# Nahuel-M/StereoVisionArray

Measured on AMD Instinct MI355X. Metric: Mdisparities/sec (W·H·D/s) at 1080p D=128, higher is better.
Workload: dtype u16

## Files before the change

### stereovisionarray_amd/csrc/sgm_common.h

```cpp
#pragma once

#include <utility>

#include "sva_device.h"
#include "sva_internal.h"
#include "sva_tuning.h"

namespace sva {
namespace sgm {

template <class F, int... S>
__device__ __forceinline__ void for_seq_impl(std::integer_sequence<int, S...>, F&& f) {
    (f(std::integral_constant<int, S>{}), ...);
}
template <int N, class F>
__device__ __forceinline__ void for_seq(F&& f) {
    for_seq_impl(std::make_integer_sequence<int, N>{}, static_cast<F&&>(f));
}

constexpr unsigned INF2 = 0x7fff7fffu;

struct PathGeom {
    int W, H, D;
    int P1, P2;
    int blk_h;
    int blk_w;
    size_t vol;
    int ckpt;
    int ns;
    size_t ckvol;
    int nsy;
    size_t ckvvol;
    int npair;
    size_t cstr, lstr, ckstr, ckvstr;
    int pair;
    int dreal;
};


typedef __amdgpu_buffer_rsrc_t rsrc_t;


constexpr int kStoreNT = 2;

__device__ __forceinline__ rsrc_t make_rsrc(const void* base, size_t bytes) {
    return __builtin_amdgcn_make_buffer_rsrc(const_cast<void*>(base), (short)0,
                                             (int)(unsigned)bytes, 0x00020000);
}

template <int NW>
struct Words {
    unsigned w[NW];
};

template <int NW, int AUX = tune::kCLoadAux>
__device__ __forceinline__ Words<NW> bload(rsrc_t r, unsigned off) {
    Words<NW> o;
    if constexpr (NW == 1) {
        o.w[0] = __builtin_amdgcn_raw_buffer_load_b32(r, off, 0, AUX);
    } else if constexpr (NW == 2) {
        auto v = __builtin_amdgcn_raw_buffer_load_b64(r, off, 0, AUX);
        o.w[0] = v[0]; o.w[1] = v[1];
    } else if constexpr (NW == 3) {
        auto v = __builtin_amdgcn_raw_buffer_load_b96(r, off, 0, AUX);
        o.w[0] = v[0]; o.w[1] = v[1]; o.w[2] = v[2];
    } else {
        auto v = __builtin_amdgcn_raw_buffer_load_b128(r, off, 0, AUX);
        o.w[0] = v[0]; o.w[1] = v[1]; o.w[2] = v[2]; o.w[3] = v[3];
    }
    return o;
}

template <int NW, int AUX = kStoreNT>
__device__ __forceinline__ void bstore(rsrc_t r, unsigned off, const unsigned (&w)[NW]) {
    if constexpr (NW == 1) {
        __builtin_amdgcn_raw_buffer_store_b32(w[0], r, off, 0, AUX);
    } else if constexpr (NW == 2) {
        typedef unsigned v2u __attribute__((ext_vector_type(2)));
        __builtin_amdgcn_raw_buffer_store_b64((v2u){w[0], w[1]}, r, off, 0, AUX);
    } else if constexpr (NW == 3) {
        typedef unsigned v3u __attribute__((ext_vector_type(3)));
        __builtin_amdgcn_raw_buffer_store_b96((v3u){w[0], w[1], w[2]}, r, off, 0, AUX);
    } else {
        typedef unsigned v4u __attribute__((ext_vector_type(4)));
        __builtin_amdgcn_raw_buffer_store_b128((v4u){w[0], w[1], w[2], w[3]}, r, off, 0, AUX);
    }
}

__device__ __forceinline__ unsigned add3(unsigned a, unsigned b, unsigned c) {
    unsigned r;
    asm("v_add3_u32 %0, %1, %2, %3" : "=v"(r) : "v"(a), "v"(b), "v"(c));
    return r;
}

template <bool DIAG>
struct Cursor {
    int x;
    unsigned off;
    __device__ __forceinline__ bool advance(int rx, unsigned stride, int W, unsigned WD) {
        off += stride;
        if constexpr (DIAG) {
            x += rx;
            const bool hi = x >= W, lo = x < 0;
            x = hi ? x - W : (lo ? x + W : x);
            off = hi ? off - WD : (lo ? off + WD : off);
            return hi || lo;
        }
        return false;
    }
};

__device__ __forceinline__ unsigned min3_u16x2(unsigned a, unsigned b, unsigned c) {
    unsigned r;
    asm("v_pk_minimum3_f16 %0, %1, %2, %3" : "=v"(r) : "v"(a), "v"(b), "v"(c));
    return r;
}

template <int NP>
__device__ __forceinline__ unsigned lane_min_u16(const unsigned (&A)[NP]) {
    unsigned mm[NP];
#pragma unroll
    for (int j = 0; j < NP; j++) mm[j] = A[j];
    int n = NP;
#pragma unroll
    for (int it = 0; it < 4; it++) {
        if (n > 1) {
            int o = 0, i = 0;
#pragma unroll
            for (int q = 0; q < 8; q++) {
                if (i + 2 < n) { mm[o++] = min3_u16x2(mm[i], mm[i + 1], mm[i + 2]); i += 3; }
                else if (i + 1 < n) { mm[o++] = as_u32(vmin2(as_v2(mm[i]), as_v2(mm[i + 1]))); i += 2; }
                else if (i < n) { mm[o++] = mm[i]; i += 1; }
            }
            n = o;
        }
    }
    const u16x2 mf = as_v2(mm[0]);
    return mf.x < mf.y ? mf.x : mf.y;
}

template <int DPL> __host__ __device__ constexpr int pair_d(int j, int h) {
    return tune::kSplitPairs ? j + h * (DPL / 2) : 2 * j + h;
}
template <int DPL> __host__ __device__ constexpr int pair_of(int e) {
    return tune::kSplitPairs ? e % (DPL / 2) : e >> 1;
}
template <int DPL> __host__ __device__ constexpr int half_of(int e) {
    return tune::kSplitPairs ? e / (DPL / 2) : e & 1;
}

template <int DPL>
__device__ __forceinline__ void words_to_pairs(const unsigned (&w)[DPL / 4], unsigned (&A)[DPL / 2]) {
    constexpr int NW = DPL / 4, NP = DPL / 2;
    if constexpr (tune::kSplitPairs != 0) {
#pragma unroll
        for (int j = 0; j < NP; j++) {
            constexpr unsigned Z = 0x0cu;
            const int el = j, eh = j + NP;
            const unsigned sel = (unsigned)(el & 3) | (Z << 8) | ((4u + (unsigned)(eh & 3)) << 16) | (Z << 24);
            A[j] = __builtin_amdgcn_perm(w[eh >> 2], w[el >> 2], sel);
        }
    } else {
#pragma unroll
        for (int q = 0; q < NW; q++) unpack4(w[q], A[2 * q], A[2 * q + 1]);
    }
}

template <int DPL>
__device__ __forceinline__ void pairs_to_words(const unsigned (&A)[DPL / 2], unsigned (&ow)[DPL / 4]) {
    constexpr int NW = DPL / 4, NP = DPL / 2;
    if constexpr (tune::kSplitPairs != 0) {
        unsigned T[NP / 2];
#pragma unroll
        for (int i = 0; i < NP / 2; i++) T[i] = __builtin_amdgcn_perm(A[2 * i + 1], A[2 * i], 0x06020400u);
        if constexpr (NP == 2) {
            ow[0] = T[0];
        } else {
#pragma unroll
            for (int q = 0; q < NW; q++) {
                const int e0 = 4 * q, e2 = 4 * q + 2;
                const int a = (e0 % NP) / 2, ha = e0 / NP, b = (e2 % NP) / 2, hb = e2 / NP;
                const unsigned sel = (unsigned)(2 * ha) | ((unsigned)(2 * ha + 1) << 8) |
                                     ((unsigned)(4 + 2 * hb) << 16) | ((unsigned)(5 + 2 * hb) << 24);
                ow[q] = __builtin_amdgcn_perm(T[b], T[a], sel);
            }
        }
    } else {
#pragma unroll
        for (int w = 0; w < NW; w++) ow[w] = pack4(A[2 * w], A[2 * w + 1]);
    }
}

struct Edges {
    unsigned X = INF2, Y = INF2;
};

template <int DPL, bool PIN = false>
__device__ __forceinline__ void sgm_step_c(const unsigned (&c)[DPL / 2], unsigned (&A)[DPL / 2],
                                           unsigned& m, unsigned (&ow)[DPL / 4], unsigned P1,
                                           unsigned P2, Edges& e) {
    constexpr int NP = DPL / 2;
    e.X = row_shr1(A[NP - 1], e.X);
    e.Y = row_shl1(A[0], e.Y);
    const unsigned X = e.X, Y = e.Y;
    unsigned lo[NP], hi[NP];
    if constexpr (tune::kSplitPairs != 0) {
#pragma unroll
        for (int j = 0; j < NP; j++) {
            lo[j] = j == 0 ? __builtin_amdgcn_alignbit(A[NP - 1], X, 16) : A[j - 1];
            hi[j] = j == NP - 1 ? __builtin_amdgcn_alignbit(Y, A[0], 16) : A[j + 1];
        }
    } else {
        unsigned M[NP];
        M[0] = __builtin_amdgcn_alignbit(A[0], X, 16);
#pragma unroll
        for (int j = 1; j < NP; j++) M[j] = __builtin_amdgcn_alignbit(A[j], A[j - 1], 16);
        const unsigned Qlast = __builtin_amdgcn_alignbit(Y, A[NP - 1], 16);
#pragma unroll
        for (int j = 0; j < NP; j++) {
            lo[j] = M[j];
            hi[j] = j < NP - 1 ? M[j + 1] : Qlast;
        }
    }
    unsigned K, mP2;
    asm("v_mul_i32_i24_e32 %0, 0xfffeffff, %1" : "=v"(K) : "v"(m));
    if constexpr (tune::kStepMadP2 != 0) {
        asm("v_mad_u32_u24 %0, %1, %2, %3" : "=&v"(mP2) : "v"(m), "s"(0x10001u), "v"(P2 * 0x10001u));
    } else {
        mP2 = P2 * 0x10001u - K;
    }
    u16x2 t[NP];
#pragma unroll
    for (int j = 0; j < NP; j++) t[j] = vmin2(as_v2(lo[j]), as_v2(hi[j]));
    unsigned tp[NP];
    if constexpr (tune::kStepAddU32 != 0) {
        const unsigned P1x2 = P1 * 0x10001u;
#pragma unroll
        for (int j = 0; j < NP; j++) tp[j] = as_u32(t[j]) + P1x2;
    } else {
#pragma unroll
        for (int j = 0; j < NP; j++) tp[j] = as_u32(t[j] + splat2(P1));
    }
#pragma unroll
    for (int j = 0; j < NP; j++) A[j] = add3(min3_u16x2(tp[j], A[j], mP2), c[j], K);
    pairs_to_words<DPL>(A, ow);
    m = row_min_u32<PIN>(lane_min_u16<NP>(A));
}

template <int DPL>
__device__ __forceinline__ void sgm_step_c(const unsigned (&c)[DPL / 2], unsigned (&A)[DPL / 2],
                                           unsigned& m, unsigned (&ow)[DPL / 4], unsigned P1,
                                           unsigned P2) {
    Edges e;
    sgm_step_c<DPL>(c, A, m, ow, P1, P2, e);
}

template <int DPL, bool PIN = false>
__device__ __forceinline__ void sgm_step(const unsigned (&cw)[DPL / 4], unsigned (&A)[DPL / 2],
                                         unsigned& m, unsigned (&ow)[DPL / 4], unsigned P1,
                                         unsigned P2, Edges& e) {
    unsigned c[DPL / 2];
    words_to_pairs<DPL>(cw, c);
    sgm_step_c<DPL, PIN>(c, A, m, ow, P1, P2, e);
}

__device__ __forceinline__ void dir_of(int r, int& rx, int& ry) {
    constexpr int T[8][2] = {{1, 0}, {-1, 0}, {0, 1}, {0, -1}, {1, 1}, {-1, -1}, {-1, 1}, {1, -1}};
    rx = T[r][0];
    ry = T[r][1];
}

template <int DPL> constexpr int pf_h() {
    return DPL == 4 ? tune::kPfH4 : DPL == 8 ? tune::kPfH8 : DPL == 12 ? tune::kPfH12 : tune::kPfH16;
}
template <int DPL> constexpr int pf_v() {
    return DPL == 4 ? tune::kPfV4 : DPL == 8 ? tune::kPfV8 : DPL == 12 ? tune::kPfV12 : tune::kPfV16;
}


template <int DPL, bool DIAG, int PF, int CKPT = 0, int SL = 0>
__device__ __forceinline__ void path_line(rsrc_t rC, rsrc_t rL, const PathGeom& g, int rx, int ry,
                                          int line, int k, rsrc_t rCK) {
    constexpr int NW = DPL / 4, NP = DPL / 2;
    const int W = g.W, H = g.H, D = g.D;
    const unsigned P1 = (unsigned)g.P1, P2 = (unsigned)g.P2;
    const int steps = ry == 0 ? W : H;
    const unsigned WD = (unsigned)W * (unsigned)D;
    const unsigned stride = (unsigned)((ry * W + rx) * D);
    int x0, y0;
    if (ry == 0) { y0 = line; x0 = rx > 0 ? 0 : W - 1; }
    else { y0 = ry > 0 ? 0 : H - 1; x0 = line; }
    Cursor<false> cc;
    cc.x = x0;
    cc.off = ((unsigned)y0 * (unsigned)W + (unsigned)x0) * (unsigned)D + (unsigned)(k * DPL);
    Cursor<false> pc = cc;
    constexpr bool STATIC_HITS = DPL <= tune::kStaticCkptHitsMaxDpl && (CKPT == 1 || CKPT == 2) &&
                                 SL > 0 && PF % (1 << SL) == 0;
    int lead = 0;
    if constexpr (STATIC_HITS) {
        constexpr int SEG = 1 << SL;
        lead = CKPT == 1 ? (rx > 0 ? 0 : (SEG - W % SEG) % SEG) : (ry > 0 ? 0 : (SEG - H % SEG) % SEG);
        pc.off -= (unsigned)lead * stride;
    }
    const int nsteps = steps + lead;
    int twc = 0, twp = 0, Tc = 0, Tp = 0;
    if constexpr (DIAG) {
        const int j = (int)((threadIdx.x >> 4) & 3);
        const int l0 = __builtin_amdgcn_readfirstlane(line - j);
        twc = twp = rx > 0 ? W - line : line + 1;
        Tc = Tp = rx > 0 ? W - l0 - 3 : l0 + 1;
    }
    const bool narrow = W < 4;

    unsigned A[NP];
#pragma unroll
    for (int j = 0; j < NP; j++) A[j] = 0u;
    unsigned m = 0u;
    Edges edges;

    Words<NW> ring[PF];
#pragma unroll
    for (int p = 0; p < PF; p++) {
        ring[p] = bload<NW>(rC, pc.off);
        if constexpr (STATIC_HITS) {
#pragma unroll
            for (int w = 0; w < NW; w++) ring[p].w[w] = p < lead ? 0u : ring[p].w[w];
        }
        pc.off += stride;
        if constexpr (DIAG) {
            if (p < PF - 1) {
                const bool w = p + 1 == twp;
                const unsigned fixed = rx > 0 ? pc.off - WD : pc.off + WD;
                pc.off = w ? fixed : pc.off;
                twp = w ? twp + W : twp;
            }
        }
    }
    if constexpr (DIAG) {
        while (Tp + 3 < PF) Tp += W;
    }

    auto step = [&](int p, bool refill, int ts) {
        unsigned cw[NW];
#pragma unroll
        for (int w = 0; w < NW; w++) cw[w] = ring[p].w[w];
        unsigned ow[NW];
        sgm_step<DPL>(cw, A, m, ow, P1, P2, edges);
        if constexpr (CKPT == 1 && STATIC_HITS) {
            constexpr int SEG = 1 << SL;
            if ((p & (SEG - 1)) == SEG - 1) {
                const int x = rx > 0 ? ts : W - 1 - (ts - lead);
                if (rx > 0 ? x + 1 < W : x > 0)
                    bstore<NW, tune::kCkptStoreAux>(rCK, ((unsigned)(y0 * g.ns + (x >> SL)) * (unsigned)D +
                                             (unsigned)(k * DPL)), ow);
            }
        } else if constexpr (CKPT == 2 && STATIC_HITS) {
            constexpr int SEG = 1 << SL;
            if ((p & (SEG - 1)) == SEG - 1) {
                const int y = ry > 0 ? ts : H - 1 - (ts - lead);
                if (ry > 0 ? y + 1 < H : y > 0)
                    bstore<NW, tune::kCkptStoreAux>(rCK, ((unsigned)((y >> SL) * W + x0) * (unsigned)D +
                                             (unsigned)(k * DPL)), ow);
            }
        } else if constexpr (CKPT == 1) {
            const int x = rx > 0 ? ts : W - 1 - ts;
            constexpr int SEG = 1 << SL;
            const bool hit = rx > 0 ? (((x + 1) & (SEG - 1)) == 0 && x + 1 < W)
                                    : ((x & (SEG - 1)) == 0 && x > 0);
            if (__builtin_expect(hit, 0))
                bstore<NW, tune::kCkptStoreAux>(rCK, ((unsigned)(y0 * g.ns + (x >> SL)) * (unsigned)D +
                                         (unsigned)(k * DPL)), ow);
        } else if constexpr (CKPT == 3) {
            const int y = ry > 0 ? ts : H - 1 - ts;
            constexpr int SEG = 1 << SL;
            const bool hit = ry > 0 ? (((y + 1) & (SEG - 1)) == 0 && y + 1 < H)
                                    : ((y & (SEG - 1)) == 0 && y > 0);
            if (__builtin_expect(hit, 0))
                bstore<NW, tune::kCkptStoreAux>(rCK, cc.off - (unsigned)(y - (y >> SL)) * WD, ow);
        } else if constexpr (CKPT == 2) {
            const int y = ry > 0 ? ts : H - 1 - ts;
            constexpr int SEG = 1 << SL;
            const bool hit = ry > 0 ? (((y + 1) & (SEG - 1)) == 0 && y + 1 < H)
                                    : ((y & (SEG - 1)) == 0 && y > 0);
            if (__builtin_expect(hit, 0))
                bstore<NW, tune::kCkptStoreAux>(rCK, ((unsigned)((y >> SL) * W + x0) * (unsigned)D +
                                         (unsigned)(k * DPL)), ow);
        } else {
            bstore<NW>(rL, cc.off, ow);
        }
        cc.off += stride;
        if constexpr (DIAG) {
            const int ec = ts + 1 - Tc;
            const int ep = ts + PF - Tp;
            const bool cev = narrow || (unsigned)ec < 4u;
            const bool pev = refill && (narrow || (unsigned)ep < 4u);
            if (__builtin_expect(cev || pev, 0)) {
                if (cev) {
                    const bool wrapped = ts + 1 == twc;
                    const unsigned fixed = rx > 0 ? cc.off - WD : cc.off + WD;
                    cc.off = wrapped ? fixed : cc.off;
                    twc = wrapped ? twc + W : twc;
#pragma unroll
                    for (int j = 0; j < NP; j++) A[j] = wrapped ? 0u : A[j];
                    m = wrapped ? 0u : m;
                    if (ec == 3) Tc += W;
                }
                if (pev) {
                    const bool wrapped = ts + PF == twp;
                    const unsigned fixed = rx > 0 ? pc.off - WD : pc.off + WD;
                    pc.off = wrapped ? fixed : pc.off;
                    twp = wrapped ? twp + W : twp;
                    if (ep == 3) Tp += W;
                }
            }
        }
        if (refill) {
            __builtin_amdgcn_sched_barrier(0);
            ring[p] = bload<NW>(rC, pc.off);
            pc.off += stride;
            __builtin_amdgcn_sched_barrier(0);
        }
    };

    int t = 0;
    for (; t + PF <= nsteps; t += PF) {
#pragma unroll
        for (int p = 0; p < PF; p++) step(p, true, t + p);
    }
#pragma unroll
    for (int p = 0; p < PF; p++)
        if (t + p < nsteps) step(p, false, t + p);
}



template <int NW>
__device__ __forceinline__ void unpack_add(const unsigned (&w)[NW], unsigned (&S)[2 * NW]) {
    unsigned a[2 * NW];
    words_to_pairs<4 * NW>(w, a);
#pragma unroll
    for (int j = 0; j < 2 * NW; j++) S[j] += a[j];
}

template <int DPL, bool PAD, bool PIN = false>
__device__ __forceinline__ void state_from_words(const Words<DPL / 4>& w, unsigned (&A)[DPL / 2],
                                                 unsigned& m, const unsigned (&padm)[DPL / 2]) {
    constexpr int NP = DPL / 2;
    words_to_pairs<DPL>(w.w, A);
    if constexpr (PAD) {
#pragma unroll
        for (int j = 0; j < NP; j++) A[j] |= padm[j] & 0x00ff00ffu;
    }
    if constexpr (tune::kStateMinTree) {
        m = row_min_u32<PIN>(lane_min_u16<NP>(A));
    } else {
        unsigned mm = 0xffffffffu;
#pragma unroll
        for (int j = 0; j < NP; j++) {
            const unsigned lo = A[j] & 0xffffu, hi = A[j] >> 16;
            mm = mm < lo ? mm : lo;
            mm = mm < hi ? mm : hi;
        }
        m = row_min_u32<PIN>(mm);
    }
}
template <int DPL, bool PAD, bool PIN = false>
__device__ __forceinline__ void load_state(rsrc_t r, unsigned off, unsigned (&A)[DPL / 2],
                                           unsigned& m, const unsigned (&padm)[DPL / 2]) {
    state_from_words<DPL, PAD, PIN>(bload<DPL / 4>(r, off), A, m, padm);
}

template <int DPL, int PF, int SL>
__device__ __forceinline__ void pair_line(rsrc_t rC, rsrc_t rE, const PathGeom& g, int rx, int line,
                                          int k, rsrc_t rCK) {
    constexpr int NW = DPL / 4, NP = DPL / 2, SEG = 1 << SL;
    path_line<DPL, true, PF, 3, SL>(rC, rC, g, rx, 1, line, k, rCK);
    asm volatile("s_waitcnt vmcnt(0)" ::: "memory");

    const int W = g.W, H = g.H;
    const unsigned uW = (unsigned)W, uD = (unsigned)g.D;
    const unsigned P1 = (unsigned)g.P1, P2 = (unsigned)g.P2;
    const unsigned lane_d = (unsigned)(k * DPL);
    const int jrow = (int)((threadIdx.x >> 4) & 3);
    const int l0 = __builtin_amdgcn_readfirstlane(line - jrow);
    const int nseg = (H + SEG - 1) >> SL;
    const int xdn = rx > 0 ? 0 : W - 1, xup = rx > 0 ? W - 1 : 0;
    unsigned padm[NP];
#pragma unroll
    for (int j = 0; j < NP; j++) {
        const int dl = k * DPL + pair_d<DPL>(j, 0), dh = k * DPL + pair_d<DPL>(j, 1);
        padm[j] = (dl >= g.dreal ? 0x0000ffffu : 0u) | (dh >= g.dreal ? 0xffff0000u : 0u);
    }
    auto wrap = [&](int x) { return x >= W ? x - W : (x < 0 ? x + W : x); };
    auto seg_x = [&](int s) {
        int xb = (l0 + rx * (s << SL)) % W;
        xb = xb < 0 ? xb + W : xb;
        int x = xb + jrow;
        x = x >= W ? x - W : x;
        x = x >= W ? x - W : x;
        x = x >= W ? x - W : x;
        return x;
    };
    struct SegLoads {
        Words<NW> c[SEG], ck;
    };
    auto issue = [&](int s, SegLoads& b) {
        int x = seg_x(s);
        if (s > 0)
            b.ck = bload<NW, 16>(rCK, ((unsigned)(s - 1) * uW + (unsigned)wrap(x - rx)) * uD + lane_d);
#pragma unroll
        for (int r = 0; r < SEG; r++) {
            b.c[r] = bload<NW>(rC, ((unsigned)((s << SL) + r) * uW + (unsigned)x) * uD + lane_d);
            x = wrap(x + rx);
        }
    };
    auto reset_if = [&](bool rs, unsigned (&A)[NP], unsigned& m) {
        if (__builtin_expect(__builtin_amdgcn_ballot_w64(rs) != 0, 0)) {
#pragma unroll
            for (int j = 0; j < NP; j++) A[j] = rs ? 0u : A[j];
            m = rs ? 0u : m;
        }
    };

    unsigned Au[NP], mu = 0u;
#pragma unroll
    for (int j = 0; j < NP; j++) Au[j] = 0u;
    Edges eu;
    SegLoads cur, nxt;
    issue(nseg - 1, cur);
    for (int s = nseg - 1; s >= 0; s--) {
        __builtin_amdgcn_sched_barrier(0);
        if (s > 0) issue(s - 1, nxt);
        __builtin_amdgcn_sched_barrier(0);
        const int y0 = s << SL;
        const int nr = H - y0 < SEG ? H - y0 : SEG;
        int x[SEG];
        x[0] = seg_x(s);
#pragma unroll
        for (int r = 1; r < SEG; r++) x[r] = wrap(x[r - 1] + rx);
        unsigned Ad[NP], md;
        Edges ed;
        if (s > 0) {
            state_from_words<DPL, true>(cur.ck, Ad, md, padm);
        } else {
#pragma unroll
            for (int j = 0; j < NP; j++) Ad[j] = 0u;
            md = 0u;
        }
        unsigned Dn[SEG][NW];
        auto down_row = [&](int r, const Words<NW>& c) {
            unsigned cp[NP], ow[NW], t[NP];
            words_to_pairs<DPL>(c.w, cp);
            sgm_step_c<DPL>(cp, Ad, md, ow, P1, P2, ed);
#pragma unroll
            for (int j = 0; j < NP; j++) t[j] = Ad[j] - cp[j];
            pairs_to_words<DPL>(t, Dn[r]);
        };
        auto up_row = [&](const Words<NW>& c, unsigned (&e)[NW]) {
            unsigned cp[NP], ow[NW], t[NP];
            words_to_pairs<DPL>(c.w, cp);
            sgm_step_c<DPL>(cp, Au, mu, ow, P1, P2, eu);
#pragma unroll
            for (int j = 0; j < NP; j++) t[j] = Au[j] - cp[j];
            pairs_to_words<DPL>(t, e);
        };
        const bool inner = rx > 0 ? x[0] >= 1 && x[0] + SEG <= W - 1 : x[0] - SEG >= 0 && x[0] <= W - 2;
        if (__builtin_expect(nr == SEG && __builtin_amdgcn_ballot_w64(!inner) == 0, 1)) {
            unsigned Up[SEG][NW];
            const unsigned off0 = ((unsigned)y0 * uW + (unsigned)x[0]) * uD + lane_d;
            const unsigned stride = (unsigned)((W + rx) * (int)uD);
            for_seq<SEG>([&](auto I) {
                constexpr int rd = decltype(I)::value, ru = SEG - 1 - rd;
                down_row(rd, cur.c[rd]);
                up_row(cur.c[ru], Up[ru]);
                if constexpr (rd >= SEG / 2) {
                    unsigned e[NW];
#pragma unroll
                    for (int w = 0; w < NW; w++) e[w] = Dn[rd][w] + Up[rd][w];
                    bstore<NW>(rE, off0 + (unsigned)rd * stride, e);
#pragma unroll
                    for (int w = 0; w < NW; w++) e[w] = Dn[ru][w] + Up[ru][w];
                    bstore<NW>(rE, off0 + (unsigned)ru * stride, e);
                }
            });
        } else {
            for_seq<SEG>([&](auto R) {
                constexpr int r = decltype(R)::value;
                if (r < nr) {
                    reset_if(x[r] == xdn, Ad, md);
                    down_row(r, cur.c[r]);
                }
            });
            for_seq<SEG>([&](auto Q) {
                constexpr int r = SEG - 1 - decltype(Q)::value;
                if (r < nr) {
                    reset_if(x[r] == xup, Au, mu);
                    unsigned e[NW];
                    up_row(cur.c[r], e);
#pragma unroll
                    for (int w = 0; w < NW; w++) e[w] += Dn[r][w];
                    bstore<NW>(rE, ((unsigned)(y0 + r) * uW + (unsigned)x[r]) * uD + lane_d, e);
                }
            });
        }
        if (s > 0) cur = nxt;
    }
}

}
}
```

### stereovisionarray_amd/csrc/sgm_paths.hip

```cpp
#include "sgm_common.h"
#include "sva_tuning.h"

namespace sva {
namespace {

using namespace sgm;

constexpr int PATH_BLOCK = 256;
constexpr int LINES_PER_BLOCK = PATH_BLOCK / 16;

template <int DPL, bool PAIR>
__global__ __launch_bounds__(PATH_BLOCK) void sgm_paths_kernel(const uint8_t* __restrict__ C,
                                                               uint8_t* __restrict__ L8,
                                                               uint8_t* __restrict__ CK,
                                                               uint8_t* __restrict__ CKV,
                                                               PathGeom g) {
    int b = blockIdx.x, r, lb, f;
    if constexpr (PAIR) {
        f = 0;
        const int npb = 2 * g.blk_w;
        if (b < npb) {
            r = 4 + 2 * (b & 1);
            lb = b >> 1;
            __builtin_amdgcn_s_setprio(3);
        } else if (b < npb + 2 * g.blk_h) {
            b -= npb;
            r = b / g.blk_h;
            lb = b - r * g.blk_h;
            __builtin_amdgcn_s_setprio(1);
        } else {
            b -= npb + 2 * g.blk_h;
            r = 2 + (b & 1);
            lb = b >> 1;
        }
    } else if (b < 2 * g.blk_h * g.npair) {
        f = b / (2 * g.blk_h);
        b -= f * 2 * g.blk_h;
        r = b / g.blk_h;
        lb = b - r * g.blk_h;
        __builtin_amdgcn_s_setprio(1);
    } else {
        b -= 2 * g.blk_h * g.npair;
        f = b / (6 * g.blk_w);
        b -= f * 6 * g.blk_w;
        r = 2 + b % 6;
        lb = b / 6;
    }
    C += (size_t)f * g.cstr;
    L8 += (size_t)f * g.lstr;
    if (g.ckpt) {
        CK += (size_t)f * g.ckstr;
        CKV += (size_t)f * g.ckvstr;
    }
    const int line = lb * LINES_PER_BLOCK + (threadIdx.x >> 4);
    const int k = threadIdx.x & 15;
    const int nlines = r < 2 ? g.H : g.W;
    if (line >= nlines) return;
    int rx, ry;
    dir_of(r, rx, ry);
    const rsrc_t rC = make_rsrc(C, g.vol);
    constexpr int SL = DPL <= 8 ? tune::kWtahvTileLog2 : tune::kWtahvTileLog2Wide;
    constexpr bool DOWN = diag_ckpt_down(DPL), UP = diag_ckpt_up(DPL);
    if constexpr (PAIR) {
        if (r >= 4) {
            const int pr = r == 4 ? 0 : 1;
            const rsrc_t rCK = make_rsrc(CKV + (size_t)(2 + pr) * g.ckvvol, g.ckvvol);
            const rsrc_t rE = make_rsrc(L8 + (size_t)pr * g.vol, g.vol);
            pair_line<DPL, pf_v<DPL>(), SL>(rC, rE, g, rx, line, k, rCK);
        } else if (r >= 2) {
            const rsrc_t rCK = make_rsrc(CKV + (size_t)(r - 2) * g.ckvvol, g.ckvvol);
            path_line<DPL, false, pf_v<DPL>(), 2, SL>(rC, rC, g, rx, ry, line, k, rCK);
        } else {
            const rsrc_t rCK = make_rsrc(CK + (size_t)r * g.ckvol, g.ckvol);
            path_line<DPL, false, pf_h<DPL>(), 1, SL>(rC, rC, g, rx, ry, line, k, rCK);
        }
    } else if (r >= 4 && g.ckpt && (ry > 0 ? DOWN : UP)) {
        const int plane = ry > 0 ? 2 + (r == 4 ? 0 : 1) : 2 + (DOWN ? 2 : 0) + (r == 5 ? 0 : 1);
        const rsrc_t rCK = make_rsrc(CKV + (size_t)plane * g.ckvvol, g.ckvvol);
        path_line<DPL, true, pf_v<DPL>(), 3, SL>(rC, rC, g, rx, ry, line, k, rCK);
    } else if (r >= 4) {
        const int slot = !g.ckpt ? r
                       : DOWN ? (r == 5 ? 0 : 1)
                       : UP ? (r == 4 ? 0 : 1)
                       : r - 4;
        const rsrc_t rL = make_rsrc(L8 + (size_t)slot * g.vol, g.vol);
        path_line<DPL, true, pf_v<DPL>()>(rC, rL, g, rx, ry, line, k, rL);
    } else if (r >= 2 && g.ckpt) {
        const rsrc_t rCK = make_rsrc(CKV + (size_t)(r - 2) * g.ckvvol, g.ckvvol);
        path_line<DPL, false, pf_v<DPL>(), 2, SL>(rC, rC, g, rx, ry, line, k, rCK);
    } else if (r >= 2) {
        const rsrc_t rL = make_rsrc(L8 + (size_t)r * g.vol, g.vol);
        path_line<DPL, false, pf_v<DPL>()>(rC, rL, g, rx, ry, line, k, rL);
    } else if (g.ckpt) {
        const rsrc_t rCK = make_rsrc(CK + (size_t)r * g.ckvol, g.ckvol);
        path_line<DPL, false, pf_h<DPL>(), 1, SL>(rC, rC, g, rx, ry, line, k, rCK);
    } else {
        const rsrc_t rL = make_rsrc(L8 + (size_t)r * g.vol, g.vol);
        path_line<DPL, false, pf_h<DPL>()>(rC, rL, g, rx, ry, line, k, rL);
    }
}

template <int DPL, bool EN>
void paths_launch(bool pair, dim3 grid, hipStream_t s, hipEvent_t start, hipEvent_t stop,
                  const uint8_t* C, uint8_t* L8, uint8_t* CK, uint8_t* CKV, const PathGeom& g) {
    if constexpr (EN) {
        if (pair) {
            hipExtLaunchKernelGGL((sgm_paths_kernel<DPL, true>), grid, dim3(PATH_BLOCK), 0, s, start,
                                  stop, 0, C, L8, CK, CKV, g);
            return;
        }
    }
    hipExtLaunchKernelGGL((sgm_paths_kernel<DPL, false>), grid, dim3(PATH_BLOCK), 0, s, start, stop,
                          0, C, L8, CK, CKV, g);
}

}

bool paths_supported(int D) { return D == 64 || D == 128 || D == 192 || D == 256; }

TileGeom tile_geom(int W, int H, int D) {
    TileGeom t;
    t.seg_log2 = D <= 128 ? tune::kWtahvTileLog2 : tune::kWtahvTileLog2Wide;
    const int seg = 1 << t.seg_log2;
    t.ntx = (W + 15) >> 4;
    t.nty = (H + seg - 1) >> t.seg_log2;
    t.nsx = (W + seg - 1) >> t.seg_log2;
    t.hck_bytes = 2 * (size_t)H * t.nsx * D;
    t.vck_bytes = 2 * (size_t)t.nty * W * D;
    const int dpl = D / 16;
    const int ndp = (diag_ckpt_down(dpl) ? 2 : 0) + (diag_ckpt_up(dpl) ? 2 : 0);
    t.dck_bytes = (size_t)ndp / 2 * t.vck_bytes;
    t.nvol = 4 - ndp;
    return t;
}

bool diag_pair_enabled(int D) {
    return (D == 64 && tune::kDiagPair4) || (D == 128 && tune::kDiagPair8) ||
           (D == 192 && tune::kDiagPair12) || (D == 256 && tune::kDiagPair16);
}

hipError_t launch_paths(Ctx& c, const uint8_t* C, int W, int H, int D, int P1, int P2,
                        uint8_t* L8, uint8_t* CK, uint8_t* CKV, int npair, bool pair, int dreal) {
    DispatchTimer t(c, "sgm_paths");
    PathGeom g;
    g.W = W; g.H = H; g.D = D; g.P1 = P1; g.P2 = P2;
    g.blk_h = (H + LINES_PER_BLOCK - 1) / LINES_PER_BLOCK;
    g.blk_w = (W + LINES_PER_BLOCK - 1) / LINES_PER_BLOCK;
    g.vol = (size_t)W * H * D;
    if ((CK == nullptr) != (CKV == nullptr)) return hipErrorInvalidValue;
    g.ckpt = CK ? 2 : 0;
    const TileGeom tg = tile_geom(W, H, D);
    g.nsy = tg.nty;
    g.ckvvol = tg.vck_bytes / 2;
    g.ns = tg.nsx;
    g.ckvol = tg.hck_bytes / 2;
    if (g.vol >= (size_t)1 << 32) return hipErrorInvalidValue;
    if (npair < 1 || (npair > 1 && !CK)) return hipErrorInvalidValue;
    g.npair = npair;
    g.cstr = g.vol;
    g.lstr = (size_t)tg.nvol * g.vol;
    g.ckstr = tg.hck_bytes;
    g.ckvstr = tg.vck_bytes + tg.dck_bytes;
    if (pair && (!CK || npair != 1 || 2 * P2 > 255 || !diag_pair_enabled(D) ||
                 tile_geom(W, H, D).nvol != 4))
        return hipErrorInvalidValue;
    g.pair = pair ? 1 : 0;
    g.dreal = dreal > 0 && dreal < D ? dreal : D;
    dim3 grid((unsigned)((2 * g.blk_h + (pair ? 4 : 6) * g.blk_w) * npair));
    t.used = true;
    switch (D) {
        case 64: paths_launch<4, tune::kDiagPair4 != 0>(pair, grid, c.stream, t.start, t.stop, C, L8, CK, CKV, g); break;
        case 128: paths_launch<8, tune::kDiagPair8 != 0>(pair, grid, c.stream, t.start, t.stop, C, L8, CK, CKV, g); break;
        case 192: paths_launch<12, tune::kDiagPair12 != 0>(pair, grid, c.stream, t.start, t.stop, C, L8, CK, CKV, g); break;
        case 256: paths_launch<16, tune::kDiagPair16 != 0>(pair, grid, c.stream, t.start, t.stop, C, L8, CK, CKV, g); break;
        default: t.used = false; return hipErrorInvalidValue;
    }
    return hipGetLastError();
}

}
```

### stereovisionarray_amd/csrc/sva_tuning.h

```cpp
#pragma once

#include <cstddef>

namespace sva {
namespace tune {

constexpr int kStepAddU32 = 1;
constexpr int kSplitPairs = 1;
constexpr int kStepMadP2 = 0;
constexpr int kPfH4 = 40, kPfV4 = 24;
constexpr int kPfH8 = 32, kPfV8 = 12;
constexpr int kPfH12 = 24, kPfV12 = 8;
constexpr int kPfH16 = 12, kPfV16 = 8;
constexpr int kCLoadAux = 0;
constexpr int kCkptStoreAux = 0;
constexpr int kStaticCkptHitsMaxDpl = 4;

constexpr int kStateMinTree = 1;

constexpr int kTileDiagDown = 0;
constexpr int kTileDiagUp = 0;
constexpr int kDiagPair4 = 0, kDiagPair8 = 1, kDiagPair12 = 0, kDiagPair16 = 0;
constexpr long long kDiagPairMinPixels = 1600000;
constexpr int kWtahvPfVolPair = 4;
constexpr int kStripRoute = 0;
constexpr int kStripTileW = 16;
constexpr int kStripCols = 128;
constexpr int kStripMinWaves = 3;
constexpr int kWtahvTileLog2 = 3;
constexpr int kWtahvTileLog2Wide = 3;
constexpr int kWtahvPfVol = 3;
constexpr int kWtahvPfVol4 = 4;
constexpr int kWtahvPfVol16 = 2;
constexpr int kWtahvInterleaveV = 0;
constexpr int kWtahvEarlyLoads = 1;
constexpr int kWtahvRowCFirst = 1;
constexpr int kWtahvKeepU16 = 3;
constexpr int kWtahvKeepU16Wide = 3;
constexpr int kWtahvPinRowMin = 1;
constexpr int kWtahvPinWta = 1;
constexpr int kWtahvSubLds = 1;
constexpr int kWtahvKeyPerm = 1;
constexpr int kWtahvSubDeferred = 1;
constexpr int kWtahvUnpackOnce = 0;
constexpr int kWtahvMinWaves = 1;
constexpr int kWtahvVSwizzle = 0;

constexpr int kBatchMaxPairs = 8;
constexpr int kBatchCostStreams = 3;
constexpr int kBatchSubFrames = 4;
constexpr size_t kBatchMaxBytes = (size_t)24 << 30;

constexpr int kPlacementTrials = 6;
constexpr size_t kPlacementMinBytes = (size_t)4 << 30;

constexpr int kCensusRows = 16;
constexpr int kCensusCostMinD = 64;
constexpr int kCensusCostRows = 8;
constexpr int kCensusCostRowsSmall = 4;
constexpr int kCensusCostMinGroups = 1536;
constexpr int kCensusCostPx4 = 64, kCensusCostPx8 = 64, kCensusCostPx12 = 64, kCensusCostPx16 = 128;
constexpr int kCostStoreNT = 1;
constexpr int kCensusCostSlotOrder = 1;
constexpr int kCensusCostWS = 0;
constexpr int kCensusCost2Lines = 8;

constexpr int kPlaneOuKB = 24;
constexpr int kPlaneWords = 1024;
constexpr int kPlaneMinBlocks = 3;
constexpr int kPlaneStageMajor = 2;
constexpr int kPlaneNoHoistDiv = 0;
constexpr int kPlanePoLds = 1;
constexpr int kPlaneSplitMin = 3;
constexpr int kPlaneSplitMax = 6;
constexpr int kPlaneSplitRounds = 4;
constexpr int kPlaneSplitInner = 2;
constexpr int kPlaneWalkRange = 1;

}
}
```

Before: 323,700.

## Split diagonal pair path work across two thread groups meeting mid-image

```diff
diff --git a/stereovisionarray_amd/csrc/sgm_common.h b/stereovisionarray_amd/csrc/sgm_common.h
--- a/stereovisionarray_amd/csrc/sgm_common.h
+++ b/stereovisionarray_amd/csrc/sgm_common.h
@@ -472,18 +472,99 @@
 
 template <int DPL, int PF, int SL>
 __device__ __forceinline__ void pair_line(rsrc_t rC, rsrc_t rE, const PathGeom& g, int rx, int line,
-                                          int k, rsrc_t rCK) {
+                                          int role, int k, rsrc_t rCK) {
     constexpr int NW = DPL / 4, NP = DPL / 2, SEG = 1 << SL;
-    path_line<DPL, true, PF, 3, SL>(rC, rC, g, rx, 1, line, k, rCK);
-    asm volatile("s_waitcnt vmcnt(0)" ::: "memory");
-
+    static_assert(PF >= SEG, "the lead steps sit in the prefetch prologue");
     const int W = g.W, H = g.H;
     const unsigned uW = (unsigned)W, uD = (unsigned)g.D;
+    const unsigned WD = uW * uD;
     const unsigned P1 = (unsigned)g.P1, P2 = (unsigned)g.P2;
     const unsigned lane_d = (unsigned)(k * DPL);
-    const int jrow = (int)((threadIdx.x >> 4) & 3);
-    const int l0 = __builtin_amdgcn_readfirstlane(line - jrow);
     const int nseg = (H + SEG - 1) >> SL;
+    const int qs = nseg >> 1;
+    const int M = qs << SL;
+    const bool up = role != 0;
+    auto wrap = [&](int x) { return x >= W ? x - W : (x < 0 ? x + W : x); };
+    auto col_of = [&](int y) {
+        const int x = (line + rx * y) % W;
+        return x < 0 ? x + W : x;
+    };
+
+    unsigned A1[NP], m1 = 0u;
+    {
+        const int n1 = M > H - M ? M : H - M;
+        const int lead = n1 - (up ? H - M : M);
+        const int ry = up ? -1 : 1, rxl = up ? -rx : rx;
+        const int yv = up ? H - 1 + lead : -lead;
+        const int xv = col_of(yv);
+        const unsigned stride = (unsigned)((ry * W + rxl) * g.D);
+        const unsigned wfix = rxl > 0 ? 0u - WD : WD;
+        unsigned coff = (unsigned)(yv * W + xv) * uD + lane_d;
+        unsigned poff = coff;
+        int twc = rxl > 0 ? W - xv : xv + 1, twp = twc;
+        const int zT = 1 - (n1 - M) - SEG, zB = H - 1 + (n1 - (H - M)) - (M + SEG);
+        const int z0 = up ? zB : zT;
+        const int zn = up ? H - (M + SEG) : M - 2 * SEG + 1;
+#pragma unroll
+        for (int j = 0; j < NP; j++) A1[j] = 0u;
+        Edges e1;
+        Words<NW> ring[PF];
+#pragma unroll
+        for (int p = 0; p < PF; p++) {
+            ring[p] = bload<NW>(rC, poff);
+#pragma unroll
+            for (int w = 0; w < NW; w++) ring[p].w[w] = p < lead ? 0u : ring[p].w[w];
+            poff += stride;
+            if (p < PF - 1) {
+                const bool wr = p + 1 == twp;
+                poff = wr ? poff + wfix : poff;
+                twp = wr ? twp + W : twp;
+            }
+        }
+        auto step = [&](int p, bool refill, int ts) {
+            unsigned cw[NW];
+#pragma unroll
+            for (int w = 0; w < NW; w++) cw[w] = ring[p].w[w];
+            unsigned ow[NW];
+            sgm_step<DPL>(cw, A1, m1, ow, P1, P2, e1);
+            if (__builtin_expect((((zT + ts) & (SEG - 1)) == 0) | (((zB - ts) & (SEG - 1)) == 0), 0)) {
+                const int zc = up ? z0 - ts : z0 + ts;
+                if ((zc & (SEG - 1)) == 0 && zc >= 0 && zc < zn) {
+                    const int y = zc + (up ? M + SEG : SEG - 1);
+                    bstore<NW, tune::kCkptStoreAux>(rCK, coff - (unsigned)(y - (y >> SL)) * WD, ow);
+                }
+            }
+            coff += stride;
+            const bool cwr = ts + 1 == twc;
+            const bool pwr = refill && ts + PF == twp;
+            if (__builtin_expect(__builtin_amdgcn_ballot_w64(cwr || pwr) != 0, 0)) {
+                coff = cwr ? coff + wfix : coff;
+                twc = cwr ? twc + W : twc;
+#pragma unroll
+                for (int j = 0; j < NP; j++) A1[j] = cwr ? 0u : A1[j];
+                m1 = cwr ? 0u : m1;
+                poff = pwr ? poff + wfix : poff;
+                twp = pwr ? twp + W : twp;
+            }
+            if (refill) {
+                __builtin_amdgcn_sched_barrier(0);
+                ring[p] = bload<NW>(rC, poff);
+                poff += stride;
+                __builtin_amdgcn_sched_barrier(0);
+            }
+        };
+        int t = 0;
+        for (; t + PF <= n1; t += PF) {
+#pragma unroll
+            for (int p = 0; p < PF; p++) step(p, true, t + p);
+        }
+#pragma unroll
+        for (int p = 0; p < PF; p++)
+            if (t + p < n1) step(p, false, t + p);
+    }
+    asm volatile("s_waitcnt vmcnt(0)" ::: "memory");
+
+    const int nit = nseg - qs;
     const int xdn = rx > 0 ? 0 : W - 1, xup = rx > 0 ? W - 1 : 0;
     unsigned padm[NP];
 #pragma unroll
@@ -491,28 +572,26 @@
         const int dl = k * DPL + pair_d<DPL>(j, 0), dh = k * DPL + pair_d<DPL>(j, 1);
         padm[j] = (dl >= g.dreal ? 0x0000ffffu : 0u) | (dh >= g.dreal ? 0xffff0000u : 0u);
     }
-    auto wrap = [&](int x) { return x >= W ? x - W : (x < 0 ? x + W : x); };
-    auto seg_x = [&](int s) {
-        int xb = (l0 + rx * (s << SL)) % W;
-        xb = xb < 0 ? xb + W : xb;
-        int x = xb + jrow;
-        x = x >= W ? x - W : x;
-        x = x >= W ? x - W : x;
-        x = x >= W ? x - W : x;
-        return x;
+    auto seg_of = [&](int i) {
+        const int s = up ? qs - 1 - i : qs + i;
+        return s < 0 ? 0 : s;
     };
+    int s8 = (SEG * rx) % W;
+    s8 = s8 < 0 ? s8 + W : s8;
+    const int ds8 = up ? -s8 : s8;
     struct SegLoads {
         Words<NW> c[SEG], ck;
     };
-    auto issue = [&](int s, SegLoads& b) {
-        int x = seg_x(s);
-        if (s > 0)
-            b.ck = bload<NW, 16>(rCK, ((unsigned)(s - 1) * uW + (unsigned)wrap(x - rx)) * uD + lane_d);
+    auto issue = [&](int s, int x, SegLoads& b) {
+        const int xa = wrap(x - rx);
 #pragma unroll
         for (int r = 0; r < SEG; r++) {
             b.c[r] = bload<NW>(rC, ((unsigned)((s << SL) + r) * uW + (unsigned)x) * uD + lane_d);
             x = wrap(x + rx);
         }
+        const bool has = up ? s > 0 : s + 1 < nseg;
+        const unsigned o = ((unsigned)(up ? s - 1 : s + 1) * uW + (unsigned)(up ? xa : x)) * uD + lane_d;
+        b.ck = bload<NW, 16>(rCK, has ? o : lane_d);
     };
     auto reset_if = [&](bool rs, unsigned (&A)[NP], unsigned& m) {
         if (__builtin_expect(__builtin_amdgcn_ballot_w64(rs) != 0, 0)) {
@@ -522,30 +601,44 @@
         }
     };
 
-    unsigned Au[NP], mu = 0u;
-#pragma unroll
-    for (int j = 0; j < NP; j++) Au[j] = 0u;
-    Edges eu;
+    unsigned Ad[NP], md = up ? 0u : m1, Au[NP], mu = up ? m1 : 0u;
+#pragma unroll
+    for (int j = 0; j < NP; j++) {
+        Ad[j] = up ? 0u : A1[j];
+        Au[j] = up ? A1[j] : 0u;
+    }
+    Edges ed, eu;
     SegLoads cur, nxt;
-    issue(nseg - 1, cur);
-    for (int s = nseg - 1; s >= 0; s--) {
+    int xs = col_of(seg_of(0) << SL), xn = xs;
+    issue(seg_of(0), xs, cur);
+    for (int i = 0; i < nit; i++) {
         __builtin_amdgcn_sched_barrier(0);
-        if (s > 0) issue(s - 1, nxt);
+        if (i + 1 < nit) {
+            xn = wrap(xs + ds8);
+            issue(seg_of(i + 1), xn, nxt);
+        }
         __builtin_amdgcn_sched_barrier(0);
+        const int s = seg_of(i);
+        const bool act = !up || i < qs;
         const int y0 = s << SL;
         const int nr = H - y0 < SEG ? H - y0 : SEG;
         int x[SEG];
-        x[0] = seg_x(s);
+        x[0] = xs;
 #pragma unroll
         for (int r = 1; r < SEG; r++) x[r] = wrap(x[r - 1] + rx);
-        unsigned Ad[NP], md;
-        Edges ed;
-        if (s > 0) {
-            state_from_words<DPL, true>(cur.ck, Ad, md, padm);
-        } else {
-#pragma unroll
-            for (int j = 0; j < NP; j++) Ad[j] = 0u;
-            md = 0u;
+        {
+            const bool has = up ? s > 0 : s + 1 < nseg;
+            unsigned Ak[NP], mk;
+            state_from_words<DPL, true>(cur.ck, Ak, mk, padm);
+#pragma unroll
+            for (int j = 0; j < NP; j++) {
+                const unsigned a = has ? Ak[j] : 0u;
+                Ad[j] = up ? a : Ad[j];
+                Au[j] = up ? Au[j] : a;
+            }
+            mk = has ? mk : 0u;
+            md = up ? mk : md;
+            mu = up ? mu : mk;
         }
         unsigned Dn[SEG][NW];
         auto down_row = [&](int r, const Words<NW>& c) {
@@ -565,7 +658,7 @@
             pairs_to_words<DPL>(t, e);
         };
         const bool inner = rx > 0 ? x[0] >= 1 && x[0] + SEG <= W - 1 : x[0] - SEG >= 0 && x[0] <= W - 2;
-        if (__builtin_expect(nr == SEG && __builtin_amdgcn_ballot_w64(!inner) == 0, 1)) {
+        if (__builtin_expect(__builtin_amdgcn_ballot_w64(!inner || nr != SEG || !act) == 0, 1)) {
             unsigned Up[SEG][NW];
             const unsigned off0 = ((unsigned)y0 * uW + (unsigned)x[0]) * uD + lane_d;
             const unsigned stride = (unsigned)((W + rx) * (int)uD);
@@ -586,14 +679,14 @@
         } else {
             for_seq<SEG>([&](auto R) {
                 constexpr int r = decltype(R)::value;
-                if (r < nr) {
+                if (r < nr && act) {
                     reset_if(x[r] == xdn, Ad, md);
                     down_row(r, cur.c[r]);
                 }
             });
             for_seq<SEG>([&](auto Q) {
                 constexpr int r = SEG - 1 - decltype(Q)::value;
-                if (r < nr) {
+                if (r < nr && act) {
                     reset_if(x[r] == xup, Au, mu);
                     unsigned e[NW];
                     up_row(cur.c[r], e);
@@ -603,9 +696,12 @@
                 }
             });
         }
-        if (s > 0) cur = nxt;
-    }
-}
-
-}
-}
+        if (i + 1 < nit) {
+            cur = nxt;
+            xs = xn;
+        }
+    }
+}
+
+}
+}
diff --git a/stereovisionarray_amd/csrc/sgm_paths.hip b/stereovisionarray_amd/csrc/sgm_paths.hip
--- a/stereovisionarray_amd/csrc/sgm_paths.hip
+++ b/stereovisionarray_amd/csrc/sgm_paths.hip
@@ -8,6 +8,7 @@
 
 constexpr int PATH_BLOCK = 256;
 constexpr int LINES_PER_BLOCK = PATH_BLOCK / 16;
+constexpr int PAIR_LINES = LINES_PER_BLOCK / 2;
 
 template <int DPL, bool PAIR>
 __global__ __launch_bounds__(PATH_BLOCK) void sgm_paths_kernel(const uint8_t* __restrict__ C,
@@ -18,7 +19,7 @@
     int b = blockIdx.x, r, lb, f;
     if constexpr (PAIR) {
         f = 0;
-        const int npb = 2 * g.blk_w;
+        const int npb = 4 * g.blk_w;
         if (b < npb) {
             r = 4 + 2 * (b & 1);
             lb = b >> 1;
@@ -52,7 +53,15 @@
         CK += (size_t)f * g.ckstr;
         CKV += (size_t)f * g.ckvstr;
     }
-    const int line = lb * LINES_PER_BLOCK + (threadIdx.x >> 4);
+    int line = lb * LINES_PER_BLOCK + (threadIdx.x >> 4);
+    int role = 0;
+    if constexpr (PAIR) {
+        if (r >= 4) {
+            const int row = (int)(threadIdx.x >> 4);
+            line = lb * PAIR_LINES + 2 * (row >> 2) + (row & 1);
+            role = (row >> 1) & 1;
+        }
+    }
     const int k = threadIdx.x & 15;
     const int nlines = r < 2 ? g.H : g.W;
     if (line >= nlines) return;
@@ -66,7 +75,7 @@
             const int pr = r == 4 ? 0 : 1;
             const rsrc_t rCK = make_rsrc(CKV + (size_t)(2 + pr) * g.ckvvol, g.ckvvol);
             const rsrc_t rE = make_rsrc(L8 + (size_t)pr * g.vol, g.vol);
-            pair_line<DPL, pf_v<DPL>(), SL>(rC, rE, g, rx, line, k, rCK);
+            pair_line<DPL, pf_v<DPL>(), SL>(rC, rE, g, rx, line, role, k, rCK);
         } else if (r >= 2) {
             const rsrc_t rCK = make_rsrc(CKV + (size_t)(r - 2) * g.ckvvol, g.ckvvol);
             path_line<DPL, false, pf_v<DPL>(), 2, SL>(rC, rC, g, rx, ry, line, k, rCK);
@@ -166,7 +175,7 @@
         return hipErrorInvalidValue;
     g.pair = pair ? 1 : 0;
     g.dreal = dreal > 0 && dreal < D ? dreal : D;
-    dim3 grid((unsigned)((2 * g.blk_h + (pair ? 4 : 6) * g.blk_w) * npair));
+    dim3 grid((unsigned)((2 * g.blk_h + 6 * g.blk_w) * npair));
     t.used = true;
     switch (D) {
         case 64: paths_launch<4, tune::kDiagPair4 != 0>(pair, grid, c.stream, t.start, t.stop, C, L8, CK, CKV, g); break;
diff --git a/stereovisionarray_amd/csrc/sva_tuning.h b/stereovisionarray_amd/csrc/sva_tuning.h
--- a/stereovisionarray_amd/csrc/sva_tuning.h
+++ b/stereovisionarray_amd/csrc/sva_tuning.h
@@ -21,7 +21,7 @@
 constexpr int kTileDiagDown = 0;
 constexpr int kTileDiagUp = 0;
 constexpr int kDiagPair4 = 0, kDiagPair8 = 1, kDiagPair12 = 0, kDiagPair16 = 0;
-constexpr long long kDiagPairMinPixels = 1600000;
+constexpr long long kDiagPairMinPixels = 1450000;
 constexpr int kWtahvPfVolPair = 4;
 constexpr int kStripRoute = 0;
 constexpr int kStripTileW = 16;
```

Measured after the change: 337,300, median of 6. 4.2% higher.
